# zhuker/lamejs

Measured on NVIDIA H100. Metric: encoded audio seconds/sec (44.1kHz stereo 128kbps CBR), higher is better.
Workload: dtype f64

## Files before the change

lamejs_b200/csrc/k_psy.cuh:

```cuda
#ifndef MP3B200_K_PSY_CUH
#define MP3B200_K_PSY_CUH
#include "mp3_device.cuh"
#include "mp3_tables.h"

#ifndef PSY_THREADS
#define PSY_THREADS 128
#endif
#define MASK_THREADS 128

struct PsyUnit {
  float eb_l[MP3_CBANDS];
  float peaks[9];
  float loudness;
  unsigned char mask_idx[MP3_CBANDS];
  unsigned char attack[4];
  unsigned char pad_;
};
struct PsyShort {
  double ecb_s[3][MP3_CBANDS];
  float eb_s[3][MP3_CBANDS];
};
struct PsyRatioDev { float en_l[22], thm_l[22], en_s[13][3], thm_s[13][3]; };

__constant__ unsigned char c_fft_rv[128];
__device__ double c_tab[9];
__device__ double c_table1[25];
__device__ double c_table2[10];
__device__ double c_table3[14];
__constant__ double c_fircoef[10];

static int psy_upload_constants() {
  static const double tab[9] = {1.0, 0.79433, 0.63096, 0.63096, 0.63096, 0.63096, 0.63096, 0.25119, 0.11749};
  static const double r1[25] = {3.3246, 3.23837, 3.15437, 3.00412, 2.86103, 2.65407, 2.46209, 2.284, 2.11879, 1.96552, 1.82335,
    1.69146, 1.56911, 1.46658, 1.37074, 1.31036, 1.25264, 1.20648, 1.16203, 1.12765, 1.09428, 1.0659, 1.03826, 1.01895, 1};
  static const double r2[10] = {1.33352, 1.35879, 1.38454, 1.39497, 1.40548, 1.3537, 1.30382, 1.22321, 1.14758, 1};
  static const double r3[14] = {2.35364, 2.29259, 2.23313, 2.12675, 2.02545, 1.87894, 1.74303, 1.61695, 1.49999, 1.39148,
    1.29083, 1.19746, 1.11084, 1.03826};
  static const double fir_half[10] = {-8.65163e-18, -0.00851586, -6.74764e-18, 0.0209036, -3.36639e-17, -0.0438162,
    -1.54175e-17, 0.0931738, -5.52212e-17, -0.313819};
  double t1[25], t2[10], t3[14], fir[10];
  for (int i = 0; i < 25; i++) t1[i] = r1[i] * r1[i];
  for (int i = 0; i < 10; i++) t2[i] = r2[i] * r2[i];
  for (int i = 0; i < 14; i++) t3[i] = r3[i] * r3[i];
  for (int i = 0; i < 10; i++) fir[i] = fir_half[i] * 2;
  if (cudaMemcpyToSymbol(c_fft_rv, MP3_FFT_RV, 128) != cudaSuccess) return -100;
  if (cudaMemcpyToSymbol(c_tab, tab, sizeof tab) != cudaSuccess) return -100;
  if (cudaMemcpyToSymbol(c_table1, t1, sizeof t1) != cudaSuccess) return -100;
  if (cudaMemcpyToSymbol(c_table2, t2, sizeof t2) != cudaSuccess) return -100;
  if (cudaMemcpyToSymbol(c_table3, t3, sizeof t3) != cudaSuccess) return -100;
  if (cudaMemcpyToSymbol(c_fircoef, fir, sizeof fir) != cudaSuccess) return -100;
  return 0;
}

struct f32w {
  float v;
  __device__ __forceinline__ operator double() const {
#ifdef PSY_ALU_WIDEN
    const unsigned u = __float_as_uint(v);
    const unsigned hi = (u & 0x7fffffffu) ? ((u & 0x80000000u) | (((u >> 3) & 0x0fffffffu) + 0x38000000u)) : u;
    return __hiloint2double((int)hi, (int)(u << 29));
#else
    return (double)v;
  }
  __device__ __forceinline__ f32w& operator=(double d) { v = (float)d; return *this; }
};
#endif

#define FHT_PAD(i) ((i) + ((i) >> 4))
__device__ __forceinline__ void fht_task(f32w* fz, int stage, int task, const double* __restrict__ tw, const int* tw_off) {
  const int k1 = 4 << (2 * stage);
  const int kx = k1 >> 1, k2 = k1 << 1, k3 = k2 + k1, k4 = k2 << 1;
  const int g = task >> (2 * stage + 1), i = task & (kx - 1);
  if (i == 0) {
    {
      const int fi = g * k4;
      double f0, f1, f2, f3;
      f1 = fz[FHT_PAD(fi + 0)] - fz[FHT_PAD(fi + k1)];
      f0 = fz[FHT_PAD(fi + 0)] + fz[FHT_PAD(fi + k1)];
      f3 = fz[FHT_PAD(fi + k2)] - fz[FHT_PAD(fi + k3)];
      f2 = fz[FHT_PAD(fi + k2)] + fz[FHT_PAD(fi + k3)];
      fz[FHT_PAD(fi + k2)] = f0 - f2;
      fz[FHT_PAD(fi + 0)] = f0 + f2;
      fz[FHT_PAD(fi + k3)] = f1 - f3;
      fz[FHT_PAD(fi + k1)] = f1 + f3;
    }
    {
      const int gi = g * k4 + kx;
      double f0, f1, f2, f3;
      f1 = fz[FHT_PAD(gi + 0)] - fz[FHT_PAD(gi + k1)];
      f0 = fz[FHT_PAD(gi + 0)] + fz[FHT_PAD(gi + k1)];
      f3 = (SQRT2_D * fz[FHT_PAD(gi + k3)]);
      f2 = (SQRT2_D * fz[FHT_PAD(gi + k2)]);
      fz[FHT_PAD(gi + k2)] = f0 - f2;
      fz[FHT_PAD(gi + 0)] = f0 + f2;
      fz[FHT_PAD(gi + k3)] = f1 - f3;
      fz[FHT_PAD(gi + k1)] = f1 + f3;
    }
    return;
  }
  const double* e = tw + 4 * (tw_off[stage] + i);
  const double c1 = e[0], s1 = e[1], c2 = e[2], s2 = e[3];
  const int fi = g * k4 + i, gi = g * k4 + k1 - i;
  double a, b, g0, f0, f1, g1, f2, g2, f3, g3;
  b = s2 * fz[FHT_PAD(fi + k1)] - c2 * fz[FHT_PAD(gi + k1)];
  a = c2 * fz[FHT_PAD(fi + k1)] + s2 * fz[FHT_PAD(gi + k1)];
  f1 = fz[FHT_PAD(fi + 0)] - a;
  f0 = fz[FHT_PAD(fi + 0)] + a;
  g1 = fz[FHT_PAD(gi + 0)] - b;
  g0 = fz[FHT_PAD(gi + 0)] + b;
  b = s2 * fz[FHT_PAD(fi + k3)] - c2 * fz[FHT_PAD(gi + k3)];
  a = c2 * fz[FHT_PAD(fi + k3)] + s2 * fz[FHT_PAD(gi + k3)];
  f3 = fz[FHT_PAD(fi + k2)] - a;
  f2 = fz[FHT_PAD(fi + k2)] + a;
  g3 = fz[FHT_PAD(gi + k2)] - b;
  g2 = fz[FHT_PAD(gi + k2)] + b;
  b = s1 * f2 - c1 * g3;
  a = c1 * f2 + s1 * g3;
  fz[FHT_PAD(fi + k2)] = f0 - a;
  fz[FHT_PAD(fi + 0)] = f0 + a;
  fz[FHT_PAD(gi + k3)] = g1 - b;
  fz[FHT_PAD(gi + k1)] = g1 + b;
  b = c1 * g2 - s1 * f3;
  a = s1 * g2 + c1 * f3;
  fz[FHT_PAD(gi + k2)] = g0 - a;
  fz[FHT_PAD(gi + 0)] = g0 + a;
  fz[FHT_PAD(fi + k3)] = f1 - b;
  fz[FHT_PAD(fi + k1)] = f1 + b;
}

__device__ __forceinline__ size_t psy_row(const StreamDesc& sd, int z, int u) { return (size_t)sd.unit_base + z + u + 1; }

template <bool F32_PCM, int NT>
__device__ __forceinline__ void psy_load_span(const Mp3Tables* __restrict__ T, const StreamDesc& sd, int ch, long long x0, double* xs) {
  using Sample = pcm_sample_t<F32_PCM>;
  const int tid = threadIdx.x;
  const int scale_applied = T->scale_applied;
  const double scale = T->scale;
  const Sample* __restrict__ pbuf = static_cast<const Sample*>(sd.pcm[ch]);
  const long long pbase = sd.pcm_base, pend = sd.pcm_end;
  constexpr int NB = (1024 + NT - 1) / NT;
  Sample v[NB];
#pragma unroll
  for (int k = 0; k < NB; k++) {
    const int j = tid + k * NT;
    const long long i = x0 + j;
    v[k] = (j < 1024 && i >= 0 && i < pend) ? __ldg(&pbuf[i - pbase]) : (Sample)0;
  }
#pragma unroll
  for (int k = 0; k < NB; k++) {
    const int j = tid + k * NT;
    if (j < 1024) xs[j] = pcm_value(v[k], scale_applied, scale);
  }
}

#ifndef PSY_MIN_BLOCKS
#define PSY_MIN_BLOCKS 12
#endif
template <bool F32_PCM>
__global__ void __launch_bounds__(PSY_THREADS, PSY_MIN_BLOCKS)
k_psy_analysis(const Mp3Tables* __restrict__ T, const StreamDesc* __restrict__ streams, PsyUnit* __restrict__ out,
               int chunk, int nchunks, int u_base) {
  const int z = blockIdx.z;
  const StreamDesc& sd = streams[z];
  const int u = (int)blockIdx.x + u_base;
  if (u >= T->mode_gr * sd.nframes) return;
  const int ch = blockIdx.y;
  const int nch = T->nch;
  const long long c = (long long)T->mode_gr * sd.frame0 + u;
  if (nchunks > 1) {
    const long long n = sd.pcm_end - sd.pcm_base;
    long long last = 576 * c - 224 + 1023 - sd.pcm_base;
    if (last > n - 1) last = n - 1;
    int mine = 0;
    while (mine < nchunks - 1 && last >= n * (mine + 1) / nchunks) mine++;
    if (mine != chunk) return;
  }
  PsyUnit* o = out + psy_row(sd, z, u) * nch + ch;
  const int tid = threadIdx.x;

  if (c < 0) {
    if (tid < MP3_CBANDS) { o->eb_l[tid] = 0.0f; o->mask_idx[tid] = 0; }
    if (tid < 9) o->peaks[tid] = 10.0f;
    if (tid == 0) o->loudness = 0.0f;
    if (tid < 4) o->attack[tid] = 0;
    return;
  }

  __shared__ __align__(16) unsigned char s_u[sizeof(double) * 1024];
  double* const xs = reinterpret_cast<double*>(s_u);
  f32s* const fe = reinterpret_cast<f32s*>(s_u);
  f32s* const s_max = reinterpret_cast<f32s*>(s_u + 2064);
  f32s* const s_avg = s_max + MP3_CBANDS;
  constexpr int PROD_HI_OFF = 2064 + 2 * 4 * MP3_CBANDS;
  static_assert(PROD_HI_OFF % 8 == 0 && PROD_HI_OFF + 256 * 8 <= (int)sizeof(s_u), "second half of the loudness terms");
  double* const prod_hi = reinterpret_cast<double*>(s_u + PROD_HI_OFF);
  __shared__ f32w wl[1024 + 64];
  __shared__ __align__(8) f32s hp[576];
  double* const prod_lo = reinterpret_cast<double*>(hp);
  static_assert(sizeof(f32s) * 576 >= 256 * 8, "first half of the loudness terms");
  __shared__ int s_peak[9];
  if (tid < 9) s_peak[tid] = __float_as_int(1.0f);

  psy_load_span<F32_PCM, PSY_THREADS>(T, sd, ch, 576 * c - 224, xs);
  __syncthreads();

  for (int i = tid; i < 576; i += PSY_THREADS) {
    const double* fb = xs + 397 + i;
    double sum1 = fb[10], sum2 = 0.0;
#pragma unroll
    for (int j = 0; j < 9; j += 2) {
      sum1 += c_fircoef[j] * (fb[j] + fb[21 - j]);
      sum2 += c_fircoef[j + 1] * (fb[j + 1] + fb[21 - j - 1]);
    }
    hp[i] = sum1 + sum2;
  }
  for (int jj = tid; jj < 128; jj += PSY_THREADS) {
    const int i = c_fft_rv[jj], x = 4 * jj;
    const float* w = T->fft_window;
    double f0, f1, f2, f3, wv;
    f0 = (double)w[i] * (double)xs[i];
    wv = (double)w[i + 0x200] * (double)xs[i + 0x200];
    f1 = f0 - wv; f0 = f0 + wv;
    f2 = (double)w[i + 0x100] * (double)xs[i + 0x100];
    wv = (double)w[i + 0x300] * (double)xs[i + 0x300];
    f3 = f2 - wv; f2 = f2 + wv;
    wl[FHT_PAD(x + 0)] = f0 + f2; wl[FHT_PAD(x + 2)] = f0 - f2; wl[FHT_PAD(x + 1)] = f1 + f3; wl[FHT_PAD(x + 3)] = f1 - f3;
    f0 = (double)w[i + 0x001] * (double)xs[i + 0x001];
    wv = (double)w[i + 0x201] * (double)xs[i + 0x201];
    f1 = f0 - wv; f0 = f0 + wv;
    f2 = (double)w[i + 0x101] * (double)xs[i + 0x101];
    wv = (double)w[i + 0x301] * (double)xs[i + 0x301];
    f3 = f2 - wv; f2 = f2 + wv;
    wl[FHT_PAD(x + 512 + 0)] = f0 + f2; wl[FHT_PAD(x + 512 + 2)] = f0 - f2; wl[FHT_PAD(x + 512 + 1)] = f1 + f3; wl[FHT_PAD(x + 512 + 3)] = f1 - f3;
  }
  __syncthreads();

  for (int i = tid; i < 576; i += PSY_THREADS) atomicMax(&s_peak[i >> 6], __float_as_int(fabsf(hp[i].v)));
#pragma unroll
  for (int stage = 0; stage < 4; stage++) {
    for (int t = tid; t < 128; t += PSY_THREADS) fht_task(wl, stage, t, T->tw, T->tw_off);
    __syncthreads();
  }

  for (int j = tid; j < 512; j += PSY_THREADS) {
    const double re = wl[FHT_PAD(512 - j)], im = wl[FHT_PAD(512 + j)];
    f32s e; e = (re * re + im * im) * 0.5;
    fe[512 - j] = (double)e;
    const int k = 512 - j;
    if (k < 512) { const double p = (double)e * (double)T->eql_w[k]; if (k < 256) prod_lo[k] = p; else prod_hi[k - 256] = p; }
  }
  if (tid == 0) { f32s t0; t0 = (double)wl[0]; t0 *= (double)t0; fe[0] = (double)t0; prod_lo[0] = (double)t0 * (double)T->eql_w[0]; }
  __syncthreads();

  const int npl = T->npart_l;
  for (int b = tid; b < npl; b += PSY_THREADS) {
    double ebb = 0, m = 0;
    const int l0 = T->line0_l[b], l1 = T->line0_l[b + 1];
    for (int j = l0; j < l1; j++) { const double el = fe[j]; ebb += el; if (m < el) m = el; }
    o->eb_l[b] = (float)ebb;
    s_max[b] = m;
    s_avg[b] = ebb * (double)T->rnumlines_l[b];
  }
  double loud = 0.0;
  if (tid == PSY_THREADS - 1) {
#pragma unroll 8
    for (int i = 0; i < 256; ++i) loud += prod_lo[i];
  }
  if (tid < 9) o->peaks[tid] = __int_as_float(s_peak[tid]);
  __syncthreads();

  for (int b = tid; b < npl; b += PSY_THREADS) {
    const int lo = b > 0 ? b - 1 : b, hi = b < npl - 1 ? b + 1 : b;
    double a = 0; double m = 0; int lines = 0;
    for (int q = lo; q <= hi; q++) {
      if (q == lo) { a = (double)s_avg[q]; m = (double)s_max[q]; }
      else { a = a + (double)s_avg[q]; if (m < (double)s_max[q]) m = (double)s_max[q]; }
      lines += T->numlines_l[q];
    }
    int k = 0;
    if (a > 0.0) {
      const double cnt = (double)(hi - lo + 1);
      a = 20.0 * (m * cnt - a) / (a * (lines - 1));
      k = js_trunc<DOM_TRUNC_MASK_IDX>(a);
      if (k > 8) k = 8;
    }
    o->mask_idx[b] = (unsigned char)k;
  }
  if (tid == PSY_THREADS - 1) {
#pragma unroll 8
    for (int i = 0; i < 256; ++i) loud += prod_hi[i];
    loud *= (1. / (14752. * 14752.) / 512);
    o->loudness = (float)loud;
  }
}


__device__ __forceinline__ bool psy_short_read(const Mp3Tables* __restrict__ T, const StreamDesc& sd,
                                               const signed char* __restrict__ bt_final, int u, int all) {
  const int n = T->mode_gr * sd.nframes;
  if (u < 0 || u >= n) return false;
  if (all || u == n - 1) return true;
  const size_t row = (size_t)(sd.unit_base + u + 1) * 2;
  return bt_final[row] == BT_SHORT || (T->nch == 2 && bt_final[row + 1] == BT_SHORT);
}

__global__ void __launch_bounds__(128)
k_psy_short_list(const Mp3Tables* __restrict__ T, const StreamDesc* __restrict__ streams, const signed char* __restrict__ bt_final,
                 int all, int2* __restrict__ list, int* __restrict__ count) {
  const int z = blockIdx.y;
  const StreamDesc& sd = streams[z];
  const int u = (int)(blockIdx.x * blockDim.x + threadIdx.x) - 1;
  if (u >= T->mode_gr * sd.nframes) return;
  if (!psy_short_read(T, sd, bt_final, u, all) && !psy_short_read(T, sd, bt_final, u + 1, all)) return;
  const int nch = T->nch;
  const int at = atomicAdd(count, nch);
  for (int ch = 0; ch < nch; ch++) list[at + ch] = make_int2(z, ((u + 1) << 1) | ch);
}

#ifndef PSY_SHORT_BLOCKS
#define PSY_SHORT_BLOCKS 8
#endif
template <bool F32_PCM>
__global__ void __launch_bounds__(PSY_THREADS)
k_psy_short(const Mp3Tables* __restrict__ T, const StreamDesc* __restrict__ streams, PsyShort* __restrict__ out,
            const int2* __restrict__ list, int* __restrict__ count) {
  const int ntasks = count[0];
  if (ntasks == 0) return;
  const int tid = threadIdx.x;
  const int nch = T->nch, nps = T->npart_s;
  __shared__ double xs[1024];
  __shared__ f32w wsh[3][256 + 16];
  __shared__ f32s fes[3][129];
  __shared__ f32s s_ebs[3][MP3_CBANDS];
  __shared__ int s_task;
  for (;;) {
    if (tid == 0) s_task = atomicAdd(count + 1, 1);
    __syncthreads();
    const int t = s_task;
    if (t >= ntasks) return;
    const int2 e = list[t];
    const int z = e.x, u = (e.y >> 1) - 1, ch = e.y & 1;
    const StreamDesc& sd = streams[z];
    const long long c = (long long)T->mode_gr * sd.frame0 + u;
    PsyShort* o = out + psy_row(sd, z, u) * nch + ch;
    if (c < 0) {
      for (int i = tid; i < 3 * MP3_CBANDS; i += PSY_THREADS) { (&o->ecb_s[0][0])[i] = 1.0; (&o->eb_s[0][0])[i] = 0.0f; }
      __syncthreads();
      continue;
    }
    psy_load_span<F32_PCM, PSY_THREADS>(T, sd, ch, 576 * c - 224, xs);
    __syncthreads();
    for (int q = tid; q < 96; q += PSY_THREADS) {
      const int b = q >> 5, j = q & 31;
      const int i = c_fft_rv[j << 2], x = 4 * j, k = 192 * (b + 1);
      const float* w = T->fft_window_s;
      const double* bx = xs + i + k;
      double f0, f1, f2, f3, wv;
      f0 = (double)w[i] * (double)bx[0];
      wv = (double)w[0x7f - i] * (double)bx[0x80];
      f1 = f0 - wv; f0 = f0 + wv;
      f2 = (double)w[i + 0x40] * (double)bx[0x40];
      wv = (double)w[0x3f - i] * (double)bx[0xc0];
      f3 = f2 - wv; f2 = f2 + wv;
      wsh[b][FHT_PAD(x + 0)] = f0 + f2; wsh[b][FHT_PAD(x + 2)] = f0 - f2; wsh[b][FHT_PAD(x + 1)] = f1 + f3; wsh[b][FHT_PAD(x + 3)] = f1 - f3;
      f0 = (double)w[i + 0x01] * (double)bx[0x01];
      wv = (double)w[0x7e - i] * (double)bx[0x81];
      f1 = f0 - wv; f0 = f0 + wv;
      f2 = (double)w[i + 0x41] * (double)bx[0x41];
      wv = (double)w[0x3e - i] * (double)bx[0xc1];
      f3 = f2 - wv; f2 = f2 + wv;
      wsh[b][FHT_PAD(x + 128 + 0)] = f0 + f2; wsh[b][FHT_PAD(x + 128 + 2)] = f0 - f2; wsh[b][FHT_PAD(x + 128 + 1)] = f1 + f3; wsh[b][FHT_PAD(x + 128 + 3)] = f1 - f3;
    }
    __syncthreads();
#pragma unroll
    for (int stage = 0; stage < 3; stage++) {
      for (int q = tid; q < 96; q += PSY_THREADS) fht_task(wsh[q >> 5], stage, q & 31, T->tw, T->tw_off);
// ... 394 lines not shown
```

lamejs_b200/csrc/mp3_encoder.cu:

```cuda
#include <cuda_runtime.h>
#include <math.h>
#include <stdio.h>
#include <algorithm>
#include <array>
#include <stdlib.h>
#include <string.h>
#include <atomic>
#include <map>
#include <mutex>
#include <string>
#include <tuple>
#include <vector>

#include "../../include/mp3b200.h"
#include "mp3_config.h"
#include "mp3_device.cuh"
#include "mp3_tables.h"
#include "k_filterbank.cuh"
#include "k_psy.cuh"
#include "k_quant.cuh"
#include "k_tag.cuh"
#include "k_resample.cuh"
#include "k_replaygain.cuh"
#include "k_stage.cuh"
// ... 384 lines not shown
  unsigned long long rg_tick = 0;
  std::map<std::tuple<const Config*, int, long long, int>, cudaGraphExec_t> exec;
  struct RgGraph { cudaGraphExec_t exec = nullptr; unsigned long long used = 0; };
  std::map<std::tuple<const Config*, bool, int, int, long long, const int*>, RgGraph> rg_exec;
  void clear_rg() { for (auto& e : rg_exec) cudaGraphExecDestroy(e.second.exec); rg_exec.clear(); }
  void clear() { for (auto& e : exec) cudaGraphExecDestroy(e.second); exec.clear(); }
};

int upload(ThreadCtx& c, void* dst, const void* src, size_t n, cudaStream_t on = nullptr) {
  if (c.arena) {
    PinnedArena& a = *c.arena;
    const size_t at = (a.used + 255) & ~(size_t)255;
    if (at + n > a.cap) { g_err = "descriptor staging overflow"; return MP3B200_ERR_CUDA; }
    memcpy(a.p + at, src, n);
    a.used = at + n;
    src = a.p + at;
  }
  CK(cudaMemcpyAsync(dst, src, n, cudaMemcpyHostToDevice, on ? on : c.st));
  return 0;
}

int wait_legacy(ThreadCtx& c) {
  if (c.session) return 0;
  CK(cudaEventRecord(c.ev_in, cudaStreamLegacy));
  CK(cudaStreamWaitEvent(c.st, c.ev_in, 0));
  return 0;
}

struct Rows { bool f32; int scale_applied; };
constexpr Rows SCALED_F32 = {true, 0};

int run_pipeline(ThreadCtx& c, Config* cfg, StreamDesc* h_streams, int S, const LaunchOpts& o,
                 const PcmArrival* arrival, Rows rows, Timings* tm) {
  cudaStream_t st = c.st;
  cudaEvent_t* ev = c.ev;
  Workspace& ws = c.ws;

  const Mp3Tables* const tab = cfg->dev[c.device];
  const int nch = cfg->host.nch;
  const bool f32_pcm = rows.f32;
  int max_frames = 0;
  long long total_frames = 0;
  int scan_rows = 0;
  int streams_with_frames = 0;
  for (int i = 0; i < S; i++) {
    StreamDesc& s = h_streams[i];
    max_frames = s.nframes > max_frames ? s.nframes : max_frames;
    total_frames += s.nframes;
    streams_with_frames += s.nframes > 0 ? 1 : 0;
    s.scan_base = scan_rows;
    scan_rows += (s.nframes + SCAN_FRAMES - 1) / SCAN_FRAMES;
  }
  int rc = wait_legacy(c);
  if (rc || (rc = upload(c, ws.streams.p, h_streams, sizeof(StreamDesc) * S))) return rc;
  if (o.carry) {
    k_handle_carry_in<<<(S + 127) / 128, 128, 0, st>>>(ws.streams.p, S, o.carry->recs, o.carry->halo_scratch);
    g_launches++;
    DBG("k_handle_carry_in");
  }
  CK(cudaEventRecord(ev[0], st));

  {
    const int nchunks = arrival ? arrival->chunks : 1;
    int u_lo[MP3_MAX_PCM_CHUNKS], u_hi[MP3_MAX_PCM_CHUNKS];
    const int G = cfg->host.mode_gr;
    for (int j = 0; j < nchunks; j++) { u_lo[j] = G * max_frames; u_hi[j] = -1; }
    if (nchunks > 1) {
      for (int s = 0; s < S; s++) {
        const StreamDesc& sd = h_streams[s];
        const long long n = sd.pcm_end - sd.pcm_base;
        for (int u = -1; u < G * sd.nframes; u++) {
          long long last = 576 * ((long long)G * sd.frame0 + u) - 224 + 1023 - sd.pcm_base;
          if (last > n - 1) last = n - 1;
          int mine = 0;
          while (mine < nchunks - 1 && last >= n * (mine + 1) / nchunks) mine++;
          if (u < u_lo[mine]) u_lo[mine] = u;
          if (u + 1 > u_hi[mine]) u_hi[mine] = u + 1;
        }
      }
    } else { u_lo[0] = -1; u_hi[0] = G * max_frames; }
    for (int j = 0; j < nchunks; j++) {
      if (arrival) CK(cudaStreamWaitEvent(st, arrival->ready[j], 0));
      if (u_hi[j] <= u_lo[j]) continue;
      dim3 gridj(u_hi[j] - u_lo[j], nch, S);
      if (f32_pcm) k_psy_analysis<true><<<gridj, PSY_THREADS, 0, st>>>(tab, ws.streams.p, ws.psy.p, j, nchunks, u_lo[j]);
      else k_psy_analysis<false><<<gridj, PSY_THREADS, 0, st>>>(tab, ws.streams.p, ws.psy.p, j, nchunks, u_lo[j]);
      g_launches++;
      DBG("k_psy_analysis");
    }
  }
  CK(cudaEventRecord(ev[1], st));
  {
    dim3 grid((cfg->host.mode_gr * max_frames + 127) / 128, 1, S);
    k_attack_prepass<<<grid, 128, 0, st>>>(tab, ws.streams.p, ws.psy.p, ws.scan_in.p);
    DBG("k_attack_prepass");
    k_stream_scan<<<S, SCAN_THREADS, 0, st>>>(tab, ws.streams.p, S, ws.scan_in.p, ws.bt_final.p, ws.bt_prev.p, ws.ath_psy.p, ws.ath_q.p, ws.scan.p);
    g_launches += 2;
    DBG("k_stream_scan");
    {
      const int G = cfg->host.mode_gr;
      const size_t smem = sizeof(double) * FB_PCM_WORDS + sizeof(float) * (FB_SLABS * 18 * FB_SLAB_STRIDE);
      void (*const k_fb)(const Mp3Tables*, const StreamDesc*, float*) = f32_pcm ? k_subband_analysis<true> : k_subband_analysis<false>;
      {
        std::lock_guard<std::mutex> lk(g_mu);
        if (!g_fb_attr_done[c.device][f32_pcm]) { CK(cudaFuncSetAttribute(k_fb, cudaFuncAttributeMaxDynamicSharedMemorySize, (int)smem)); g_fb_attr_done[c.device][f32_pcm] = true; }
      }
      cudaLaunchConfig_t lc = {};
      lc.gridDim = dim3((G * max_frames + 1 + FB_SLABS - 1) / FB_SLABS, nch, S);
      lc.blockDim = dim3(FB_THREADS); lc.dynamicSmemBytes = smem; lc.stream = st;
      cudaLaunchAttribute at[1];
      at[0].id = cudaLaunchAttributeProgrammaticStreamSerialization;
      at[0].val.programmaticStreamSerializationAllowed = 1;
      lc.attrs = at; lc.numAttrs = 1;
      CK(cudaLaunchKernelEx(&lc, k_fb, tab, (const StreamDesc*)ws.streams.p, ws.slab.p));
      g_launches++;
      DBG("k_subband_analysis");
    }
  }
  CK(cudaEventRecord(ev[2], st));
  if (o.force_bt) {
    const long long units = (long long)cfg->host.mode_gr * total_frames;
    std::vector<signed char> bt((size_t)units * 2, 0);
    for (long long u = 0; u < units; u++)
      for (int c = 0; c < nch; c++) bt[u * 2 + c] = (signed char)o.force_bt[u * nch + c];
    CK(cudaMemcpyAsync(ws.bt_final.p, bt.data(), bt.size(), cudaMemcpyHostToDevice, st));
    CK(cudaStreamSynchronize(st));
  }
  {
    CK(cudaMemsetAsync(ws.short_count.p, 0, 2 * sizeof(int), st));
    dim3 grid((cfg->host.mode_gr * max_frames + 1 + 127) / 128, S);
    k_psy_short_list<<<grid, 128, 0, st>>>(tab, ws.streams.p, ws.bt_final.p, o.all_short ? 1 : 0, ws.short_list.p, ws.short_count.p);
    DBG("k_psy_short_list");
    int sms = 132;
    CK(cudaDeviceGetAttribute(&sms, cudaDevAttrMultiProcessorCount, c.device));
    const long long tasks = ((long long)cfg->host.mode_gr * total_frames + S) * nch;
    const int blocks = (int)std::min<long long>(std::max<long long>(tasks, 1), (long long)sms * PSY_SHORT_BLOCKS);
    if (f32_pcm) k_psy_short<true><<<blocks, PSY_THREADS, 0, st>>>(tab, ws.streams.p, ws.psy_s.p, ws.short_list.p, ws.short_count.p);
    else k_psy_short<false><<<blocks, PSY_THREADS, 0, st>>>(tab, ws.streams.p, ws.psy_s.p, ws.short_list.p, ws.short_count.p);
    g_launches += 2;
    DBG("k_psy_short");
  }
  {
    dim3 grid(cfg->host.mode_gr * max_frames + 1, 1, S);
    k_psy_masking<<<grid, MASK_THREADS, 0, st>>>(tab, ws.streams.p, ws.psy.p, ws.psy_s.p, ws.bt_prev.p, ws.bt_final.p,
                                                 o.all_short ? 1 : 0, ws.ath_psy.p, ws.ratio.p);
    g_launches++;
    DBG("k_psy_masking");
  }
  CK(cudaEventRecord(ev[3], st));
  {
    dim3 grid((cfg->host.mode_gr * max_frames + FB_G - 1) / FB_G, nch, S);
    k_mdct<<<grid, FB_G * 32, 0, st>>>(tab, ws.streams.p, ws.slab.p, ws.bt_final.p, ws.xr.p);
    g_launches++;
    DBG("k_mdct");
  }
  CK(cudaEventRecord(ev[4], st));
  int passes = 0;
  if (!o.stop_after_mdct) {
    QuantBuffers qb;
    qb.xr = ws.xr.p; qb.ratio = ws.ratio.p; qb.bt = ws.bt_final.p; qb.ath_q = ws.ath_q.p; qb.qs = ws.qstate.p; qb.ginfo = ws.ginfo.p;
    qb.l3enc = ws.l3enc.p; qb.xrq = ws.xrq.p; qb.xrpow = ws.xrpow.p; qb.neg = ws.neg.p; qb.prep = ws.prep.p; qb.list = ws.dirty.p; qb.counter = ws.counter.p;
    qb.over_budget = ws.refusals.p + 1;
    QuantLoop dloop;
    cudaGraphExec_t* cached = nullptr;
    if (o.loops) {
      LoopGraphs& lg = *o.loops;
      if (lg.generation != ws.generation()) { lg.clear(); lg.generation = ws.generation(); }
      cached = &lg.exec[std::make_tuple((const Config*)cfg, S, total_frames, max_frames)];
      dloop.capture = lg.capture; dloop.st = ws.refusals.p + 2; dloop.exec = *cached;
// ... 1162 lines not shown
  return debug_replaygain(channels, samplerate, kbps, flags, left, right, nsamples, win_sums, win_idx, nwin_cap, hist, title_db, stats);
}
}

extern "C" {

int mp3b200_wav_read_header(const uint8_t* data, int64_t len, mp3b200_wav_header* out) {
  if (!out || len < 0 || (len > 0 && !data)) return MP3B200_ERR_HANDLE;
  long long off = 0, dl = 0; int ch = 0; unsigned sr = 0;
  const int rc = mp3_wav_read_header(data, len, &off, &dl, &ch, &sr);
  out->data_offset = off; out->data_len = dl; out->channels = ch; out->sample_rate = sr;
  return rc;
}

int mp3b200_debug_music_crc(const uint8_t* d_buf, const int64_t* off, const int64_t* len, int nranges, uint32_t* crc, float* ms) {
  if (nranges < 0 || (nranges > 0 && (!d_buf || !off || !len || !crc))) return MP3B200_ERR_HANDLE;
  int dev = 0;
  { std::lock_guard<std::mutex> lk(g_mu); dev = g_device; int rc = ensure_device(dev); if (rc) return rc; }
  int rc = t_ctx.use(dev);
  if (rc || (rc = crc_tables_on(dev)) || (rc = wait_legacy(t_ctx))) return rc;
  std::vector<long long> at(off, off + nranges), l(len, len + nranges);
  for (long long& a : at) a += (long long)(uintptr_t)d_buf;
  for (int run = 0; run < (ms ? 2 : 1); run++) {
    if (run) CK(cudaEventRecord(t_ctx.ev[0], t_ctx.st));
    if ((rc = queue_music_crc(t_ctx, at, l))) return rc;
    if (nranges > 0) CK(cudaMemcpyAsync(crc, t_ctx.crc.p, sizeof(uint32_t) * (size_t)nranges, cudaMemcpyDeviceToHost, t_ctx.st));
    if (run) CK(cudaEventRecord(t_ctx.ev[1], t_ctx.st));
    CK(cudaStreamSynchronize(t_ctx.st));
    CK(cudaGetLastError());
  }
  if (ms) CK(cudaEventElapsedTime(ms, t_ctx.ev[0], t_ctx.ev[1]));
  return 0;
}

int mp3b200_get_vbr_tag(const uint8_t* frame, int64_t len, mp3b200_vbr_tag_data* out) {
  if (!out || len < 0 || (len > 0 && !frame)) return MP3B200_ERR_HANDLE;
  Mp3VbrTagData t;
  const int rc = mp3_tag_parse(frame, len, &t);
  out->h_id = t.h_id; out->samprate = t.samprate; out->flags = t.flags; out->frames = t.frames; out->bytes = t.bytes;
  out->vbr_scale = t.vbr_scale; out->headersize = t.headersize; out->enc_delay = t.enc_delay; out->enc_padding = t.enc_padding;
  memcpy(out->toc, t.toc, 100);
  return rc;
}

int mp3b200_crc16_combine(int crc_a, int crc_b, int64_t len_b) {
  if (len_b < 0) return MP3B200_ERR_HANDLE;
  return (int)crc_append((unsigned)crc_a & 0xffffu, (unsigned)crc_b & 0xffffu, (unsigned long long)len_b, crc_host().pow);
}

int mp3b200_lametag_size(int channels, int samplerate, int kbps) {
  return mp3b200_lametag_size_ex(channels, samplerate, kbps, 0);
}

int mp3b200_lametag_size_ex(int channels, int samplerate, int kbps, int flags) {
  const Config* c = host_config(channels, samplerate, kbps, flags);
  if (!c) return MP3B200_ERR_CONFIG;
  return c->tag.fits ? c->tag.frame_bytes : 0;
}

int mp3b200_lametag_build(int channels, int samplerate, int kbps, int64_t nframes, int64_t music_bytes, int music_crc, int encoder_padding,
                          uint8_t* buf, int cap) {
  return build_lametag(channels, samplerate, kbps, 0, nframes, music_bytes, music_crc, encoder_padding, 0, buf, cap);
}

int mp3b200_lametag_build_ex(int channels, int samplerate, int kbps, int flags, int64_t nframes, int64_t music_bytes, int music_crc,
                             int encoder_padding, int radio_gain, uint8_t* buf, int cap) {
  return build_lametag(channels, samplerate, kbps, flags, nframes, music_bytes, music_crc, encoder_padding,
                       mp3_radio_gain_field(radio_gain), buf, cap);
}

}

#include "mp3_session.inc"
#include "mp3_handle.inc"
#include "mp3_session_handles.inc"

#ifdef Q_TASKSTAT
extern "C" int mp3b200_debug_taskstat(int* out, int rows) {
  if (rows > (1 << 16)) rows = 1 << 16;
  return cudaMemcpyFromSymbol(out, g_taskstat, sizeof(int) * 8 * (size_t)rows) == cudaSuccess ? 0 : -1;
}
#endif

#ifdef MP3_DOMAIN_CHECK
extern "C" int mp3b200_debug_domain_hits(unsigned long long* out, int cap) {
  if (cap < DOM_NSITES) return DOM_NSITES;
  if (cudaDeviceSynchronize() != cudaSuccess) return -1;
  if (cudaMemcpyFromSymbol(out, g_domain_hits, sizeof(unsigned long long) * DOM_NSITES) != cudaSuccess) return -1;
  static const unsigned long long zero[DOM_NSITES] = {};
  return cudaMemcpyToSymbol(g_domain_hits, zero, sizeof zero) == cudaSuccess ? DOM_NSITES : -1;
}
#endif
```

Baseline: 58430.

## Process two granules per psy block sharing one overlapping PCM span

The psychoacoustic analysis kernel now handles two consecutive granules per block, with 64 threads per granule. Both granules read one shared PCM span, so the overlapping samples are loaded once. The change also vectorizes the highpass FIR with double2 loads and computes each peak with a warp max reduction instead of shared atomics. It replaces the bit-reversal constant table with __brev and checks that table on the host, and lowers the min-blocks launch bound. Shared memory per block grows, and per-unit partition work now relies on one thread per partition within 64 threads.

```diff
diff --git a/lamejs_b200/csrc/k_psy.cuh b/lamejs_b200/csrc/k_psy.cuh
--- a/lamejs_b200/csrc/k_psy.cuh
+++ b/lamejs_b200/csrc/k_psy.cuh
@@ -38,6 +38,11 @@
     1.29083, 1.19746, 1.11084, 1.03826};
   static const double fir_half[10] = {-8.65163e-18, -0.00851586, -6.74764e-18, 0.0209036, -3.36639e-17, -0.0438162,
     -1.54175e-17, 0.0931738, -5.52212e-17, -0.313819};
+  for (int j = 0; j < 128; j++) {
+    int r = 0;
+    for (int bit = 0; bit < 7; bit++) r |= (j >> bit & 1) << (6 - bit);
+    if (MP3_FFT_RV[j] != 2 * r) return -100;
+  }
   double t1[25], t2[10], t3[14], fir[10];
   for (int i = 0; i < 25; i++) t1[i] = r1[i] * r1[i];
   for (int i = 0; i < 10; i++) t2[i] = r2[i] * r2[i];
@@ -130,7 +135,7 @@
 
 __device__ __forceinline__ size_t psy_row(const StreamDesc& sd, int z, int u) { return (size_t)sd.unit_base + z + u + 1; }
 
-template <bool F32_PCM, int NT>
+template <bool F32_PCM, int NT, int N = 1024>
 __device__ __forceinline__ void psy_load_span(const Mp3Tables* __restrict__ T, const StreamDesc& sd, int ch, long long x0, double* xs) {
   using Sample = pcm_sample_t<F32_PCM>;
   const int tid = threadIdx.x;
@@ -138,138 +143,208 @@
   const double scale = T->scale;
   const Sample* __restrict__ pbuf = static_cast<const Sample*>(sd.pcm[ch]);
   const long long pbase = sd.pcm_base, pend = sd.pcm_end;
-  constexpr int NB = (1024 + NT - 1) / NT;
+  constexpr int NB = (N + NT - 1) / NT;
   Sample v[NB];
 #pragma unroll
   for (int k = 0; k < NB; k++) {
     const int j = tid + k * NT;
     const long long i = x0 + j;
-    v[k] = (j < 1024 && i >= 0 && i < pend) ? __ldg(&pbuf[i - pbase]) : (Sample)0;
+    v[k] = (j < N && i >= 0 && i < pend) ? __ldg(&pbuf[i - pbase]) : (Sample)0;
   }
 #pragma unroll
   for (int k = 0; k < NB; k++) {
     const int j = tid + k * NT;
-    if (j < 1024) xs[j] = pcm_value(v[k], scale_applied, scale);
-  }
-}
-
+    if (j < N) xs[j] = pcm_value(v[k], scale_applied, scale);
+  }
+}
+
+#ifndef PSY_UNITS
+#define PSY_UNITS 2
+#endif
+#ifndef PSY_UNIT_THREADS
+#define PSY_UNIT_THREADS 64
+#endif
+#define PSY_A_THREADS (PSY_UNITS * PSY_UNIT_THREADS)
 #ifndef PSY_MIN_BLOCKS
-#define PSY_MIN_BLOCKS 12
-#endif
+#define PSY_MIN_BLOCKS 8
+#endif
+static_assert(PSY_UNIT_THREADS >= 64 && PSY_UNIT_THREADS % 32 == 0, "one thread per long partition of each unit");
+
+#ifdef PSY_PHASESTAT
+#define PSY_STAT_EVERY 16
+#define PSY_STAT_ROWS 4096
+#define PSY_STAT_COLS 13
+__device__ long long g_psystat[PSY_STAT_ROWS][PSY_STAT_COLS];
+#define PSY_CLOCK(col, who) do { if (stat_row >= 0 && (who)) g_psystat[stat_row][col] = clock64(); } while (0)
+#else
+#define PSY_CLOCK(col, who) do { } while (0)
+#endif
+
+__device__ __forceinline__ bool psy_unit_in_slice(const StreamDesc& sd, long long c, int chunk, int nchunks) {
+  if (nchunks <= 1) return true;
+  const long long n = sd.pcm_end - sd.pcm_base;
+  long long last = 576 * c - 224 + 1023 - sd.pcm_base;
+  if (last > n - 1) last = n - 1;
+  int mine = 0;
+  while (mine < nchunks - 1 && last >= n * (mine + 1) / nchunks) mine++;
+  return mine == chunk;
+}
+
 template <bool F32_PCM>
-__global__ void __launch_bounds__(PSY_THREADS, PSY_MIN_BLOCKS)
+__global__ void __launch_bounds__(PSY_A_THREADS, PSY_MIN_BLOCKS)
 k_psy_analysis(const Mp3Tables* __restrict__ T, const StreamDesc* __restrict__ streams, PsyUnit* __restrict__ out,
                int chunk, int nchunks, int u_base) {
+  constexpr int U = PSY_UNITS, NT = PSY_A_THREADS;
   const int z = blockIdx.z;
   const StreamDesc& sd = streams[z];
-  const int u = (int)blockIdx.x + u_base;
-  if (u >= T->mode_gr * sd.nframes) return;
+  const int u0 = (int)blockIdx.x * U + u_base;
   const int ch = blockIdx.y;
   const int nch = T->nch;
-  const long long c = (long long)T->mode_gr * sd.frame0 + u;
-  if (nchunks > 1) {
-    const long long n = sd.pcm_end - sd.pcm_base;
-    long long last = 576 * c - 224 + 1023 - sd.pcm_base;
-    if (last > n - 1) last = n - 1;
-    int mine = 0;
-    while (mine < nchunks - 1 && last >= n * (mine + 1) / nchunks) mine++;
-    if (mine != chunk) return;
-  }
-  PsyUnit* o = out + psy_row(sd, z, u) * nch + ch;
+  const int nunits = T->mode_gr * sd.nframes;
+  const long long c0 = (long long)T->mode_gr * sd.frame0 + u0;
   const int tid = threadIdx.x;
-
-  if (c < 0) {
-    if (tid < MP3_CBANDS) { o->eb_l[tid] = 0.0f; o->mask_idx[tid] = 0; }
-    if (tid < 9) o->peaks[tid] = 10.0f;
-    if (tid == 0) o->loudness = 0.0f;
-    if (tid < 4) o->attack[tid] = 0;
-    return;
-  }
-
-  __shared__ __align__(16) unsigned char s_u[sizeof(double) * 1024];
-  double* const xs = reinterpret_cast<double*>(s_u);
-  f32s* const fe = reinterpret_cast<f32s*>(s_u);
-  f32s* const s_max = reinterpret_cast<f32s*>(s_u + 2064);
-  f32s* const s_avg = s_max + MP3_CBANDS;
-  constexpr int PROD_HI_OFF = 2064 + 2 * 4 * MP3_CBANDS;
-  static_assert(PROD_HI_OFF % 8 == 0 && PROD_HI_OFF + 256 * 8 <= (int)sizeof(s_u), "second half of the loudness terms");
-  double* const prod_hi = reinterpret_cast<double*>(s_u + PROD_HI_OFF);
-  __shared__ f32w wl[1024 + 64];
-  __shared__ __align__(8) f32s hp[576];
-  double* const prod_lo = reinterpret_cast<double*>(hp);
-  static_assert(sizeof(f32s) * 576 >= 256 * 8, "first half of the loudness terms");
-  __shared__ int s_peak[9];
-  if (tid < 9) s_peak[tid] = __float_as_int(1.0f);
-
-  psy_load_span<F32_PCM, PSY_THREADS>(T, sd, ch, 576 * c - 224, xs);
+  PsyUnit* const o0 = out + psy_row(sd, z, u0) * nch + ch;
+#ifdef PSY_PHASESTAT
+  const int stat_row = (z == 0 && ch == 0 && blockIdx.x % PSY_STAT_EVERY == 0 && blockIdx.x / PSY_STAT_EVERY < PSY_STAT_ROWS)
+                       ? (int)blockIdx.x / PSY_STAT_EVERY : -1;
+#endif
+  PSY_CLOCK(0, tid == 0);
+
+  unsigned act = 0;
+#pragma unroll
+  for (int k = 0; k < U; k++) {
+    const int u = u0 + k;
+    if (u >= nunits || !psy_unit_in_slice(sd, c0 + k, chunk, nchunks)) continue;
+    if (c0 + k < 0) {
+      PsyUnit* o = o0 + k * nch;
+      if (tid < MP3_CBANDS) { o->eb_l[tid] = 0.0f; o->mask_idx[tid] = 0; }
+      if (tid < 9) o->peaks[tid] = 10.0f;
+      if (tid == 0) o->loudness = 0.0f;
+      if (tid < 4) o->attack[tid] = 0;
+      continue;
+    }
+    act |= 1u << k;
+  }
+  if (act == 0) return;
+
+  constexpr int SPAN = 576 * (U - 1) + 1024;
+  constexpr int HP_OFF = SPAN * 8;
+  constexpr int POST = 2064 + 2 * 4 * MP3_CBANDS + 512 * 8;
+  constexpr int A_BYTES = HP_OFF + U * 576 * 4 > U * POST ? HP_OFF + U * 576 * 4 : U * POST;
+  static_assert(POST % 16 == 0 && (2064 + 2 * 4 * MP3_CBANDS) % 8 == 0, "per-unit layout of region A");
+  __shared__ __align__(16) unsigned char s_a[A_BYTES];
+  double* const xs = reinterpret_cast<double*>(s_a);
+  f32s* const hp = reinterpret_cast<f32s*>(s_a + HP_OFF);
+  __shared__ f32w wl[U][1024 + 64];
+
+  psy_load_span<F32_PCM, NT, SPAN>(T, sd, ch, 576 * c0 - 224, xs);
   __syncthreads();
-
-  for (int i = tid; i < 576; i += PSY_THREADS) {
-    const double* fb = xs + 397 + i;
-    double sum1 = fb[10], sum2 = 0.0;
+  PSY_CLOCK(1, tid == 0);
+
+  for (int p = tid; p < U * 288; p += NT) {
+    double v[24];
+    const double2* src = reinterpret_cast<const double2*>(xs + 396 + 2 * p);
 #pragma unroll
-    for (int j = 0; j < 9; j += 2) {
-      sum1 += c_fircoef[j] * (fb[j] + fb[21 - j]);
-      sum2 += c_fircoef[j + 1] * (fb[j + 1] + fb[21 - j - 1]);
-    }
-    hp[i] = sum1 + sum2;
-  }
-  for (int jj = tid; jj < 128; jj += PSY_THREADS) {
-    const int i = c_fft_rv[jj], x = 4 * jj;
+    for (int t = 0; t < 12; t++) { const double2 d = src[t]; v[2 * t] = d.x; v[2 * t + 1] = d.y; }
+#pragma unroll
+    for (int r = 0; r < 2; r++) {
+      const double* fb = v + 1 + r;
+      double sum1 = fb[10], sum2 = 0.0;
+#pragma unroll
+      for (int j = 0; j < 9; j += 2) {
+        sum1 += c_fircoef[j] * (fb[j] + fb[21 - j]);
+        sum2 += c_fircoef[j + 1] * (fb[j + 1] + fb[21 - j - 1]);
+      }
+      hp[2 * p + r] = sum1 + sum2;
+    }
+  }
+  for (int q = tid; q < U * 128; q += NT) {
+    const int k = q >> 7, p = q & 127, jj = (int)(__brev((unsigned)p) >> 25);
+    const int i = 2 * p, x = 4 * jj;
     const float* w = T->fft_window;
+    const double* xu = xs + 576 * k;
+    f32w* const y = wl[k];
     double f0, f1, f2, f3, wv;
-    f0 = (double)w[i] * (double)xs[i];
-    wv = (double)w[i + 0x200] * (double)xs[i + 0x200];
+    f0 = (double)w[i] * (double)xu[i];
+    wv = (double)w[i + 0x200] * (double)xu[i + 0x200];
     f1 = f0 - wv; f0 = f0 + wv;
-    f2 = (double)w[i + 0x100] * (double)xs[i + 0x100];
-    wv = (double)w[i + 0x300] * (double)xs[i + 0x300];
+    f2 = (double)w[i + 0x100] * (double)xu[i + 0x100];
+    wv = (double)w[i + 0x300] * (double)xu[i + 0x300];
     f3 = f2 - wv; f2 = f2 + wv;
-    wl[FHT_PAD(x + 0)] = f0 + f2; wl[FHT_PAD(x + 2)] = f0 - f2; wl[FHT_PAD(x + 1)] = f1 + f3; wl[FHT_PAD(x + 3)] = f1 - f3;
-    f0 = (double)w[i + 0x001] * (double)xs[i + 0x001];
-    wv = (double)w[i + 0x201] * (double)xs[i + 0x201];
+    y[FHT_PAD(x + 0)] = f0 + f2; y[FHT_PAD(x + 2)] = f0 - f2; y[FHT_PAD(x + 1)] = f1 + f3; y[FHT_PAD(x + 3)] = f1 - f3;
+    f0 = (double)w[i + 0x001] * (double)xu[i + 0x001];
+    wv = (double)w[i + 0x201] * (double)xu[i + 0x201];
     f1 = f0 - wv; f0 = f0 + wv;
-    f2 = (double)w[i + 0x101] * (double)xs[i + 0x101];
-    wv = (double)w[i + 0x301] * (double)xs[i + 0x301];
+    f2 = (double)w[i + 0x101] * (double)xu[i + 0x101];
+    wv = (double)w[i + 0x301] * (double)xu[i + 0x301];
     f3 = f2 - wv; f2 = f2 + wv;
-    wl[FHT_PAD(x + 512 + 0)] = f0 + f2; wl[FHT_PAD(x + 512 + 2)] = f0 - f2; wl[FHT_PAD(x + 512 + 1)] = f1 + f3; wl[FHT_PAD(x + 512 + 3)] = f1 - f3;
+    y[FHT_PAD(x + 512 + 0)] = f0 + f2; y[FHT_PAD(x + 512 + 2)] = f0 - f2; y[FHT_PAD(x + 512 + 1)] = f1 + f3; y[FHT_PAD(x + 512 + 3)] = f1 - f3;
   }
   __syncthreads();
-
-  for (int i = tid; i < 576; i += PSY_THREADS) atomicMax(&s_peak[i >> 6], __float_as_int(fabsf(hp[i].v)));
+  PSY_CLOCK(2, tid == 0);
+
+  for (int sb = tid >> 5; sb < 9 * U; sb += NT / 32) {
+    const int lane = tid & 31;
+    const unsigned m = __reduce_max_sync(0xffffffffu, max(__float_as_uint(fabsf(hp[64 * sb + lane].v)),
+                                                          __float_as_uint(fabsf(hp[64 * sb + 32 + lane].v))));
+    const int k = sb / 9;
+    if (lane == 0 && (act >> k & 1)) o0[k * nch].peaks[sb - 9 * k] = __uint_as_float(max(m, __float_as_uint(1.0f)));
+  }
 #pragma unroll
   for (int stage = 0; stage < 4; stage++) {
-    for (int t = tid; t < 128; t += PSY_THREADS) fht_task(wl, stage, t, T->tw, T->tw_off);
+    for (int t = tid; t < U * 128; t += NT) fht_task(wl[t >> 7], stage, t & 127, T->tw, T->tw_off);
     __syncthreads();
-  }
-
-  for (int j = tid; j < 512; j += PSY_THREADS) {
-    const double re = wl[FHT_PAD(512 - j)], im = wl[FHT_PAD(512 + j)];
+    PSY_CLOCK(3 + stage, tid == 0);
+  }
+
+  for (int q = tid; q < U * 512; q += NT) {
+    const int k = q >> 9, j = q & 511;
+    unsigned char* const pk = s_a + k * POST;
+    f32s* const fe = reinterpret_cast<f32s*>(pk);
+    double* const prod = reinterpret_cast<double*>(pk + 2064 + 2 * 4 * MP3_CBANDS);
+    const double re = wl[k][FHT_PAD(512 - j)], im = wl[k][FHT_PAD(512 + j)];
     f32s e; e = (re * re + im * im) * 0.5;
     fe[512 - j] = (double)e;
-    const int k = 512 - j;
-    if (k < 512) { const double p = (double)e * (double)T->eql_w[k]; if (k < 256) prod_lo[k] = p; else prod_hi[k - 256] = p; }
-  }
-  if (tid == 0) { f32s t0; t0 = (double)wl[0]; t0 *= (double)t0; fe[0] = (double)t0; prod_lo[0] = (double)t0 * (double)T->eql_w[0]; }
+    if (j > 0) prod[512 - j] = (double)e * (double)T->eql_w[512 - j];
+  }
+  if (tid < U) {
+    unsigned char* const pk = s_a + tid * POST;
+    f32s* const fe = reinterpret_cast<f32s*>(pk);
+    double* const prod = reinterpret_cast<double*>(pk + 2064 + 2 * 4 * MP3_CBANDS);
+    f32s t0; t0 = (double)wl[tid][0]; t0 *= (double)t0; fe[0] = (double)t0; prod[0] = (double)t0 * (double)T->eql_w[0];
+  }
   __syncthreads();
-
+  PSY_CLOCK(7, tid == 0);
+
+  const int k = tid / PSY_UNIT_THREADS, b = tid % PSY_UNIT_THREADS;
   const int npl = T->npart_l;
-  for (int b = tid; b < npl; b += PSY_THREADS) {
+  unsigned char* const pk = s_a + k * POST;
+  f32s* const fe = reinterpret_cast<f32s*>(pk);
+  f32s* const s_max = reinterpret_cast<f32s*>(pk + 2064);
+  f32s* const s_avg = s_max + MP3_CBANDS;
+  const double* const prod = reinterpret_cast<const double*>(pk + 2064 + 2 * 4 * MP3_CBANDS);
+  const bool mine = act >> k & 1;
+  PsyUnit* const o = o0 + k * nch;
+  if (b < npl) {
     double ebb = 0, m = 0;
     const int l0 = T->line0_l[b], l1 = T->line0_l[b + 1];
     for (int j = l0; j < l1; j++) { const double el = fe[j]; ebb += el; if (m < el) m = el; }
-    o->eb_l[b] = (float)ebb;
+    if (mine) o->eb_l[b] = (float)ebb;
     s_max[b] = m;
     s_avg[b] = ebb * (double)T->rnumlines_l[b];
   }
+  const bool chain = b == PSY_UNIT_THREADS - 1 && mine;
   double loud = 0.0;
-  if (tid == PSY_THREADS - 1) {
+  if (chain) {
 #pragma unroll 8
-    for (int i = 0; i < 256; ++i) loud += prod_lo[i];
-  }
-  if (tid < 9) o->peaks[tid] = __int_as_float(s_peak[tid]);
+    for (int i = 0; i < 256; ++i) loud += prod[i];
+  }
+  PSY_CLOCK(11, chain && k == 0);
+  PSY_CLOCK(8, tid == 0);
   __syncthreads();
-
-  for (int b = tid; b < npl; b += PSY_THREADS) {
+  PSY_CLOCK(9, tid == 0);
+
+  if (b < npl) {
     const int lo = b > 0 ? b - 1 : b, hi = b < npl - 1 ? b + 1 : b;
     double a = 0; double m = 0; int lines = 0;
     for (int q = lo; q <= hi; q++) {
@@ -277,21 +352,23 @@
       else { a = a + (double)s_avg[q]; if (m < (double)s_max[q]) m = (double)s_max[q]; }
       lines += T->numlines_l[q];
     }
-    int k = 0;
+    int kk = 0;
     if (a > 0.0) {
       const double cnt = (double)(hi - lo + 1);
       a = 20.0 * (m * cnt - a) / (a * (lines - 1));
-      k = js_trunc<DOM_TRUNC_MASK_IDX>(a);
-      if (k > 8) k = 8;
-    }
-    o->mask_idx[b] = (unsigned char)k;
-  }
-  if (tid == PSY_THREADS - 1) {
+      kk = js_trunc<DOM_TRUNC_MASK_IDX>(a);
+      if (kk > 8) kk = 8;
+    }
+    if (mine) o->mask_idx[b] = (unsigned char)kk;
+  }
+  PSY_CLOCK(10, tid == 0);
+  if (chain) {
 #pragma unroll 8
-    for (int i = 0; i < 256; ++i) loud += prod_hi[i];
+    for (int i = 256; i < 512; ++i) loud += prod[i];
     loud *= (1. / (14752. * 14752.) / 512);
     o->loudness = (float)loud;
   }
+  PSY_CLOCK(12, chain && k == 0);
 }
 
 
diff --git a/lamejs_b200/csrc/mp3_encoder.cu b/lamejs_b200/csrc/mp3_encoder.cu
--- a/lamejs_b200/csrc/mp3_encoder.cu
+++ b/lamejs_b200/csrc/mp3_encoder.cu
@@ -490,9 +490,9 @@
     for (int j = 0; j < nchunks; j++) {
       if (arrival) CK(cudaStreamWaitEvent(st, arrival->ready[j], 0));
       if (u_hi[j] <= u_lo[j]) continue;
-      dim3 gridj(u_hi[j] - u_lo[j], nch, S);
-      if (f32_pcm) k_psy_analysis<true><<<gridj, PSY_THREADS, 0, st>>>(tab, ws.streams.p, ws.psy.p, j, nchunks, u_lo[j]);
-      else k_psy_analysis<false><<<gridj, PSY_THREADS, 0, st>>>(tab, ws.streams.p, ws.psy.p, j, nchunks, u_lo[j]);
+      dim3 gridj((u_hi[j] - u_lo[j] + PSY_UNITS - 1) / PSY_UNITS, nch, S);
+      if (f32_pcm) k_psy_analysis<true><<<gridj, PSY_A_THREADS, 0, st>>>(tab, ws.streams.p, ws.psy.p, j, nchunks, u_lo[j]);
+      else k_psy_analysis<false><<<gridj, PSY_A_THREADS, 0, st>>>(tab, ws.streams.p, ws.psy.p, j, nchunks, u_lo[j]);
       g_launches++;
       DBG("k_psy_analysis");
     }
@@ -1821,6 +1821,13 @@
 }
 #endif
 
+#ifdef PSY_PHASESTAT
+extern "C" int mp3b200_debug_psystat(long long* out, int rows) {
+  if (rows > PSY_STAT_ROWS) rows = PSY_STAT_ROWS;
+  return cudaMemcpyFromSymbol(out, g_psystat, sizeof(long long) * PSY_STAT_COLS * (size_t)rows) == cudaSuccess ? rows : -1;
+}
+#endif
+
 #ifdef MP3_DOMAIN_CHECK
 extern "C" int mp3b200_debug_domain_hits(unsigned long long* out, int cap) {
   if (cap < DOM_NSITES) return DOM_NSITES;
```

Measured after the change: 61700 (median of 6 runs). 1.06x the previous value.
